# zhang-tao-whu/DVIS_Plus

Hardware: AMD Instinct MI355X
Metric: frames/sec DVIS++ R50 offline, 720p T=30 synthetic (higher is better)
Workload: dtype f32 (storage, accumulation, results; the segmenter's dense layers - R50 convolutions from 128 channels on, pixel-decoder projections and FPN output convolution, the deformable encoder's projections and FFN, the decoder's key / value projections - multiply each fp32 operand as two f16 terms on the f1

## Files before the change

### dvis_plus_amd/csrc/gemm_x3.hip

```cpp
#define DVIS_X3_DMA_MUBUF 1
#include "dvis_common.h"
#include "x3_common.h"

#include <stdlib.h>

namespace {

template <int KS>
__device__ __forceinline__ void load_x(const float *x, int64_t ldx, int64_t row, int g, float s, h8 *xh, h8 *xl,
                                       const float *addp = nullptr) {
  const float *p = x + row * ldx + 8 * g;
  f4 raw[2 * KS];
#pragma unroll
  for (int S = 0; S < KS; ++S) raw[2 * S] = *(const f4 *)(p + 16 * S), raw[2 * S + 1] = *(const f4 *)(p + 16 * S + 4);
  if (addp != nullptr) {
#pragma unroll
    for (int S = 0; S < KS; ++S) raw[2 * S] += *(const f4 *)(addp + 16 * S), raw[2 * S + 1] += *(const f4 *)(addp + 16 * S + 4);
  }
#pragma unroll
  for (int S = 0; S < KS; ++S) split8(raw[2 * S], raw[2 * S + 1], s, xh[S], xl[S]);
}

__device__ __forceinline__ void store_block(char *scr, int lane, const f4 *v, float *dst, int64_t ld, int rows_valid,
                                            const float *radd = nullptr, int64_t ldr = 0) {
// ... 16 lines not shown
  const float *res;
  int64_t ldres;
  const float *gamma, *beta;
  float eps;
  const float *pos;
  int64_t pos_rows;
  float *out, *out2;
  int64_t ldo;
  float inv;
  int relu;
  const float *radd;
  int *flag;
  int tag;
};

template <int NB, bool LN, bool EX = false>
__device__ __forceinline__ void epilogue(f16v *acc, const EpiArgs &e, const float *cb, const float *cg, const float *cbeta, char *scr,
                                         int lane, int64_t tok0, int64_t M, int col0 = 0) {
  const int j = lane & 31, g = lane >> 5;
  const int64_t tok = tok0 + j < M ? tok0 + j : M - 1;
  const int rows_valid = M - tok0 < 32 ? (int)(M - tok0) : 32;
  constexpr int N = 32 * NB;
  float mean = 0.f, rstd = 1.f;
  if constexpr (LN) {
    const float *rp = e.res + tok * e.ldres + 4 * g;
    f4 r[2][4];
    auto fetch = [&](int nb, f4 *dst) {
#pragma unroll
      for (int q = 0; q < 4; ++q) dst[q] = *(const f4 *)(rp + 32 * nb + 8 * q);
    };
    fetch(0, r[0]);
    float sum = 0.f;
#pragma unroll
// ... 25 lines not shown
    rstd = rsqrtf(sq * (1.f / N) + e.eps);
  }
  float chk = 0.f;
  const float *pr = nullptr;
  f4 pv[2][4];
  auto fetch_pos = [&](int nb, f4 *dst) {
#pragma unroll
    for (int q = 0; q < 4; ++q) dst[q] = *(const f4 *)(pr + 32 * nb + 8 * q);
  };
  if constexpr (LN) {
    if (e.pos != nullptr) {
      pr = e.pos + (tok % e.pos_rows) * N + 4 * g;
      fetch_pos(0, pv[0]);
    }
  }
#pragma unroll
  for (int nb = 0; nb < NB; ++nb) {
    f4 v[4];
    if constexpr (LN) {
      if (e.pos != nullptr && nb + 1 < NB) fetch_pos(nb + 1, pv[(nb + 1) & 1]);
    }
#pragma unroll
    for (int q = 0; q < 4; ++q) {
      const int n = 32 * nb + 8 * q + 4 * g;
      if constexpr (LN) {
        const f4 ga = *(const f4 *)(cg + n), be = *(const f4 *)(cbeta + n);
#pragma unroll
        for (int i = 0; i < 4; ++i) v[q][i] = (acc[nb][4 * q + i] - mean) * rstd * ga[i] + be[i];
      } else {
        const f4 b = *(const f4 *)(cb + n);
#pragma unroll
        for (int i = 0; i < 4; ++i) {
          const float t = acc[nb][4 * q + i] * e.inv + b[i];
          chk = __builtin_fmaf(t, 0.f, chk);
          if constexpr (EX)
            v[q][i] = e.relu == 1 ? x3_relu(t) : e.relu == 2 ? 0.5f * t * (1.f + erff(t * 0.70710678118654752440f)) : t;
          else
            v[q][i] = e.relu ? x3_relu(t) : t;
        }
      }
    }
    if constexpr (!EX)
      store_block(scr, lane, v, e.out + tok0 * e.ldo + col0 + 32 * nb, e.ldo, rows_valid);
    else
      store_block(scr, lane, v, e.out + tok0 * e.ldo + col0 + 32 * nb, e.ldo, rows_valid,
                  e.radd ? e.radd + tok0 * e.ldres + col0 + 32 * nb : nullptr, e.ldres);
    if constexpr (LN) {
      if (e.pos != nullptr) {
#pragma unroll
        for (int q = 0; q < 4; ++q) v[q] += pv[nb & 1][q];
        store_block(scr, lane, v, e.out2 + tok0 * e.ldo + 32 * nb, e.ldo, rows_valid);
      }
    }
  }
  if constexpr (!LN) {
// ... 153 lines not shown
          products(stage, acc, xh + 2 * half, xl + 2 * half);
        }
      }
      if (tok0 < M) epilogue<NB, LN, EX>(acc, e, cst + pass * 32 * NB, cst + ntot, cst + ntot + 32 * NB, scr, lane, tok0, M, pass * 32 * NB);
    }
    rowp = nrowp;
  }
}

struct FfnArgs {
  const float *b1;
  float inv1, hscale;
  int HB;
};

__global__ __launch_bounds__(kThreads) void x3_ffn_kernel(const float *__restrict__ x, int64_t ldx, int64_t M,
                                                          const void *__restrict__ wp, float xscale, FfnArgs f, EpiArgs e) {
  extern __shared__ __attribute__((aligned(1024))) char lds[];
  constexpr int KS = 16;
  const int wave = threadIdx.x >> 6, lane = threadIdx.x & 63, j = lane & 31, g = lane >> 5;
  const int64_t ntiles = (M + kTileTok - 1) / kTileTok;
  const int64_t my = blockIdx.x < ntiles ? (ntiles - blockIdx.x + gridDim.x - 1) / gridDim.x : 0;
  const int per_tile = 8 * f.HB;
  Ring<8> ring;
  ring.start(wp, lds, per_tile, (int)(my * per_tile), wave, lane);
  char *scr = lds + kStages * Ring<8>::kItemBytes + wave * kScratch;
  float *b1s = (float *)(lds + kStages * Ring<8>::kItemBytes + kWaves * kScratch);
  for (int i = threadIdx.x; i < 128 * f.HB; i += kThreads) b1s[i] = f.b1[i];
  float *cst = b1s + 128 * f.HB;
  for (int i = threadIdx.x; i < 256; i += kThreads) cst[i] = e.bias[i], cst[256 + i] = e.gamma[i], cst[512 + i] = e.beta[i];
  __syncthreads();
  for (int64_t tile = blockIdx.x; tile < ntiles; tile += gridDim.x) {
    const int64_t tok0 = tile * kTileTok + wave * 32;
    const int64_t row = tok0 + j < M ? tok0 + j : M - 1;
    h8 xh[KS], xl[KS];
    load_x<KS>(x, ldx, row, g, xscale, xh, xl);
    f16v acc2[8];
#pragma unroll
    for (int nb = 0; nb < 8; ++nb)
#pragma unroll
      for (int i = 0; i < 16; ++i) acc2[nb][i] = 0.f;
    for (int hb = 0; hb < f.HB; ++hb) {
      f16v acc1[4];
#pragma unroll
      for (int t = 0; t < 4; ++t)
// ... 22 lines not shown
        mma_item<16, 1, 8>(stage, lane, acc1 + c, xh, xl, [&](int i) { ring.piece(i); }, [&](int t) {
          if (c > 0) convert(c - 1, t);
        });
      }
#pragma unroll
      for (int c = 0; c < 4; ++c) {
        const char *stage = ring.wait(false);
        ring.begin_periodic();
        if (c == 0) {
          mma_item<2, 8, 8>(stage, lane, acc2, hh, hl, [&](int i) { ring.piece(i); }, [&](int t) { convert(3, t); });
        } else {
          mma_item<2, 8, 8>(stage, lane, acc2, hh + 2 * c, hl + 2 * c, [&](int i) { ring.piece(i); });
        }
      }
    }
    if (tok0 < M) epilogue<8, true>(acc2, e, cst, cst + 256, cst + 512, scr, lane, tok0, M);
  }
}

__global__ void x3_ffn_pack_kernel(const float *w1, int64_t ldw1, const float *w2, int64_t ldw2, int H, float s1, float s2,
                                   _Float16 *out, int64_t fragments) {
  const int64_t idx = (int64_t)blockIdx.x * blockDim.x + threadIdx.x;
  if (idx >= fragments) return;
  const int lane = idx & 63;
  int64_t t = idx >> 6;
  const int fr = t & 15;
  t >>= 4;
  const int item = t & 7, hb = t >> 3;
  _Float16 *o = out + (((int64_t)hb * 8 + item) * 16 + fr) * 1024 + lane * 8;
  if (item < 4) {
    x3_pack_fragment(w1, ldw1, H, 256, 128 * hb + 32 * item + (lane & 31), 0, fr, lane >> 5, s1, o, o + 512);
  } else {
    const int s = fr >> 3, nb = fr & 7;
    x3_pack_fragment(w2, ldw2, 256, H, 32 * nb + (lane & 31), 1, 8 * hb + 2 * (item - 4) + s, lane >> 5, s2, o, o + 512);
  }
}

int x3_grid(int64_t ntiles) {
  const int cus = dvis_x3_persistent_cus();
  return (int)(ntiles < cus ? ntiles : cus);
}

float x3_pow2(int e) { return ldexpf(1.f, e); }

template <typename Kern, typename... Args>
int x3_launch(Kern kern, DvisLdsOptIn *opted, size_t lds_bytes, int64_t M, hipStream_t st, const char *what, Args... args) {
  const int rc = dvis_lds_opt_in((const void *)kern, lds_bytes, opted, what);
  if (rc != DVIS_OK) return rc;
  const int64_t ntiles = (M + kTileTok - 1) / kTileTok;
  hipLaunchKernelGGL(kern, dim3(x3_grid(ntiles)), dim3(kThreads), lds_bytes, st, args...);
// ... 202 lines not shown
DVIS_EXPORT int64_t dvis_x3_ffn_packed_bytes(int K, int H, int N) {
  if (K != 256 || N != 256 || H <= 0 || H % 128 != 0 || H > 4096) return -1;
  return (int64_t)(H / 128) * 8 * Ring<8>::kItemBytes;
}

DVIS_EXPORT int dvis_x3_ffn_pack(const float *w1, int64_t ldw1, const float *w2, int64_t ldw2, int K, int H, int N, int w1exp,
                                 int w2exp, void *packed, void *stream) {
  DVIS_REQUIRE(w1 && w2 && packed, "dvis_x3_ffn_pack: null operand");
  DVIS_REQUIRE(dvis_x3_ffn_packed_bytes(K, H, N) > 0, "dvis_x3_ffn_pack: needs K = N = 256, H %% 128 == 0 (K %d, H %d, N %d)", K, H, N);
  const int64_t fragments = (int64_t)(H / 128) * 8 * 16 * 64;
  hipLaunchKernelGGL(x3_ffn_pack_kernel, dim3((unsigned)((fragments + 255) / 256)), dim3(256), 0, (hipStream_t)stream, w1, ldw1,
                     w2, ldw2, H, x3_pow2(w1exp), x3_pow2(w2exp), (_Float16 *)packed, fragments);
  return dvis_check_launch("dvis_x3_ffn_pack");
}

DVIS_EXPORT int dvis_x3_ffn_ln(const float *x, int64_t ldx, int64_t M, int K, int H, int N, const void *wp, int xexp, int w1exp,
                               int hexp, int w2exp, const float *b1, const float *b2, const float *gamma, const float *beta,
                               float eps, const float *pos, int64_t pos_rows, float *out, float *out2, int64_t ldo,
                               void *stream) {
  DVIS_REQUIRE(dvis_x3_ffn_packed_bytes(K, H, N) > 0, "dvis_x3_ffn_ln: needs K = N = 256, H %% 128 == 0 (K %d, H %d, N %d)", K, H, N);
  DVIS_REQUIRE(b1 && b2 && gamma && beta, "dvis_x3_ffn_ln: biases, gamma, beta are required");
  DVIS_REQUIRE(pos == nullptr || (out2 && pos_rows > 0 && (uintptr_t)pos % 16 == 0 && (uintptr_t)out2 % 16 == 0),
               "dvis_x3_ffn_ln: pos needs out2, pos_rows > 0 and 16-byte alignment");
  const int rc = x3_check_common(x, ldx, M, wp, out, ldo);
  if (rc != DVIS_OK) return rc;
  if (M == 0) return DVIS_OK;
  EpiArgs e = {};
  e.bias = b2, e.res = x, e.ldres = ldx, e.gamma = gamma, e.beta = beta, e.eps = eps, e.pos = pos, e.pos_rows = pos_rows;
  e.out = out, e.out2 = out2, e.ldo = ldo, e.inv = x3_pow2(-(hexp + w2exp));
  const X3Guard gd = dvis_x3_guard();
  e.flag = gd.flag, e.tag = gd.tag;
  FfnArgs f = {b1, x3_pow2(-(xexp + w1exp)), x3_pow2(hexp), H / 128};
  static DvisLdsOptIn opted;
  return x3_launch(x3_ffn_kernel, &opted, kStages * Ring<8>::kItemBytes + kWaves * kScratch + (size_t)(H + 3 * 256) * 4, M,
                   (hipStream_t)stream, "dvis_x3_ffn_ln", x, ldx, M, wp, x3_pow2(xexp), f, e);
}
```

### dvis_plus_amd/functions.py

```python
import collections
import ctypes
import math
import os
import threading

import torch
from torch.autograd import Function
from torch.autograd.function import once_differentiable

from . import cpu_ops, derived, native
from .cpu_ops import ms_deform_attn_core_pytorch


def _torch_path(op, x, why):
    if os.environ.get("DVIS_STRICT", "1") != "0" and x.is_cuda and not torch.is_grad_enabled():
        raise RuntimeError(f"DVIS_STRICT: {op} would run its torch formulation on a GPU tensor ({why}; shape "
                           f"{tuple(x.shape)}, dtype {x.dtype}, contiguous {x.is_contiguous()})")


class no_autocast:

    def __enter__(self):
        import contextlib
        self._stack = contextlib.ExitStack()
# ... 1406 lines not shown
            ctypes.c_void_p(x2.data_ptr()), ldx, x2.shape[0], K, ctypes.c_void_p(buf.data_ptr()), N,
            X3_XEXP if xexp is None else xexp, wexp, native.dev_ptr(bias.detach(), "bias"), ctypes.c_void_p(r2.data_ptr()), ldr,
            native.dev_ptr(norm.weight.detach(), "gamma"), native.dev_ptr(norm.bias.detach(), "beta"), float(norm.eps),
            None if pos is None else ctypes.c_void_p(pos.data_ptr()), pos_rows, ctypes.c_void_p(out.data_ptr()),
            None if out2 is None else ctypes.c_void_p(out2.data_ptr()), N, native.stream_ptr(x.device)), "dvis_x3_linear_ln")
    return out if out2 is None else (out, out2)


def x3_ffn_ok(x, lin1, lin2):
    K, H, N = lin1.weight.shape[1], lin1.weight.shape[0], lin2.weight.shape[0]
    return (x.is_cuda and x.dtype == torch.float32 and not torch.is_grad_enabled() and x.shape[-1] == K
            and lin2.weight.shape[1] == H and lin1.bias is not None and lin2.bias is not None
            and native.lib().dvis_x3_ffn_packed_bytes(K, H, N) > 0)


def x3_ffn_ln(x, lin1, lin2, norm, pos=None, xexp=None, hexp=None):
    w1, w2 = lin1.weight, lin2.weight
    H, K = w1.shape
    N = w2.shape[0]
    x2, ldx = _x3_rows(x, "x")

    def make():
        a, b = w1.detach().contiguous(), w2.detach().contiguous()
        e1, e2 = _x3_wexp(a), _x3_wexp(b)
        buf = torch.empty(native.lib().dvis_x3_ffn_packed_bytes(K, H, N), dtype=torch.uint8, device=a.device)
        with torch.cuda.device(a.device):
            native.check(native.lib().dvis_x3_ffn_pack(ctypes.c_void_p(a.data_ptr()), K, ctypes.c_void_p(b.data_ptr()), H, K, H,
                                                       N, e1, e2, ctypes.c_void_p(buf.data_ptr()),
                                                       native.stream_ptr(a.device)), "dvis_x3_ffn_pack")
        return buf, e1, e2
    buf, e1, e2 = _x3_cache(w1, [w1, w2], make, kind="ffn")
    out = torch.empty((*x.shape[:-1], N), dtype=torch.float32, device=x.device)
    pos, pos_rows, out2 = _x3_pos(pos, x, N)
    with torch.cuda.device(x.device):
        native.check(native.lib().dvis_x3_ffn_ln(
            ctypes.c_void_p(x2.data_ptr()), ldx, x2.shape[0], K, H, N, ctypes.c_void_p(buf.data_ptr()),
            X3_XEXP if xexp is None else xexp, e1, X3_XEXP if hexp is None else hexp, e2,
            native.dev_ptr(lin1.bias.detach(), "b1"), native.dev_ptr(lin2.bias.detach(), "b2"),
            native.dev_ptr(norm.weight.detach(), "gamma"), native.dev_ptr(norm.bias.detach(), "beta"), float(norm.eps),
            None if pos is None else ctypes.c_void_p(pos.data_ptr()), pos_rows, ctypes.c_void_p(out.data_ptr()),
            None if out2 is None else ctypes.c_void_p(out2.data_ptr()), N, native.stream_ptr(x.device)), "dvis_x3_ffn_ln")
    return out if out2 is None else (out, out2)


def maps_to_tokens(maps, affines=None, pos=None):
    affines = affines or [None] * len(maps)
    N, C = maps[0].shape[:2]
    if not all(m.is_cuda and m.dtype == torch.float32 and m.is_contiguous() for m in maps) or torch.is_grad_enabled():
        _torch_path("maps_to_tokens", maps[0], "needs contiguous fp32 NCHW maps")
        maps = [m if a is None else m * a[0].view(N, C, 1, 1) + a[1].view(N, C, 1, 1) for m, a in zip(maps, affines)]
        out = torch.cat([m.flatten(2).transpose(1, 2) for m in maps], 1)
        return out if pos is None else (out, out + pos.reshape(1, -1, C))
    S = sum(m.shape[2] * m.shape[3] for m in maps)
    out = torch.empty((N, S, C), dtype=torch.float32, device=maps[0].device)
    out_pos = pp = None
    if pos is not None:
# ... 1089 lines not shown
```

### dvis_plus_amd/native.py

```python
import ctypes
import os

import torch

_HERE = os.path.dirname(os.path.abspath(__file__))
LIB_PATH = os.environ.get("DVIS_HIP_LIB") or os.path.join(_HERE, "lib", "libdvis_hip.so")

F32, F64, F16, BF16 = 0, 1, 2, 3
_DTYPE = {torch.float32: F32, torch.float64: F64, torch.float16: F16, torch.bfloat16: BF16}

_c = ctypes
_i, _i64, _p, _f = _c.c_int, _c.c_int64, _c.c_void_p, _c.c_float

SIGNATURES = {
    "dvis_last_error": (_c.c_char_p, []),
    "dvis_version": (_i, []),
    "dvis_msda_forward": (_i, [_i, _p, _p, _p, _p, _p, _i, _i, _i, _i, _i, _i, _i, _p, _p]),
    "dvis_msda_backward": (_i, [_i, _p, _p, _p, _p, _p, _p, _i, _i, _i, _i, _i, _i, _i, _p, _p, _p, _p]),
    "dvis_msda_backward_det_ws_bytes": (_i64, [_i, _i, _i, _i]),
    "dvis_msda_backward_det": (_i, [_p, _p, _p, _p, _p, _p, _i, _i, _i, _i, _i, _i, _i, _p, _p, _p, _p, _p]),
    "dvis_msda_fused_forward": (_i, [_p, _p, _p, _p, _i, _p, _i64, _p, _i64, _i, _i, _i, _i, _i, _i, _i, _p, _p, _p]),
    "dvis_msda_fused_forward_pos": (_i, [_p, _p, _p, _p, _i, _p, _i64, _p, _i64, _p, _p, _i64, _i, _i, _i, _i, _i, _i, _i,
                                         _p, _p, _p]),
    "dvis_msda_fused_forward_h": (_i, [_i, _p, _p, _p, _p, _i, _p, _i64, _p, _i64, _i, _i, _i, _i, _i, _i, _i, _p, _p, _p]),
# ... 71 lines not shown
    "dvis_x3_tile_linear_qkv": (_i, [_p, _i64, _i64, _i, _p, _i, _i, _i, _p, _i, _i, _f, _p, _p]),
    "dvis_attention_x3_packed": (_i, [_p, _p, _p, _i, _i, _i, _p]),
    "dvis_x3_rows_image_bytes": (_i64, [_i64, _i]),
    "dvis_x3_rows_image": (_i, [_p, _i64, _i64, _i, _i, _p, _p]),
    "dvis_layernorm_rows_image": (_i, [_p, _p, _p, _i64, _i, _f, _i, _p, _p]),
    "dvis_x3_tile_pack_order": (_i, [_p, _i64, _i, _i, _i, _i, _p, _p]),
    "dvis_x3_tile_linear_image": (_i, [_p, _i64, _i, _p, _i, _i, _i, _p, _i, _p, _i64, _p, _i64, _p, _i, _p]),
    "dvis_x3_tile_linear_qkv_image": (_i, [_p, _i64, _i, _p, _i, _i, _i, _p, _i, _i, _f, _p, _p]),
    "dvis_attention_x3_packed_image": (_i, [_p, _p, _i, _i, _i, _i, _p]),
    "dvis_x3_tile_linear": (_i, [_p, _i64, _i64, _i, _p, _i, _i, _i, _p, _i, _p, _i64, _p, _i64, _p]),
    "dvis_x3_linear_res": (_i, [_p, _i64, _i64, _i, _p, _i, _i, _i, _p, _i, _p, _i64, _p, _i64, _p]),
    "dvis_x3_linear_add": (_i, [_p, _i64, _i64, _i, _p, _i, _i, _i, _p, _i64, _p, _i, _p, _i64, _p]),
    "dvis_x3_linear_ln": (_i, [_p, _i64, _i64, _i, _p, _i, _i, _i, _p, _p, _i64, _p, _p, _f, _p, _i64, _p, _p, _i64, _p]),
    "dvis_x3_ffn_packed_bytes": (_i64, [_i, _i, _i]),
    "dvis_x3_ffn_pack": (_i, [_p, _i64, _p, _i64, _i, _i, _i, _i, _i, _p, _p]),
    "dvis_x3_ffn_ln": (_i, [_p, _i64, _i64, _i, _i, _i, _p, _i, _i, _i, _i, _p, _p, _p, _p, _f, _p, _i64, _p, _p, _i64, _p]),
    "dvis_conv1x1_x3_supported": (_i, [_i, _i, _i64, _i64, _i64]),
    "dvis_conv1x1_x3_packed_bytes": (_i64, [_i, _i]),
    "dvis_conv1x1_x3_pack": (_i, [_p, _i, _i, _i, _p, _p]),
    "dvis_conv_x3_gn_fold_supported": (_i, [_i, _i, _i64]),
    "dvis_conv1x1_x3": (_i, [_p, _p, _p, _p, _p, _i, _i, _i, _i, _i, _i, _i, _i, _i, _p, _p, _p, _i, _p]),
    "dvis_conv1x1_x3_dual": (_i, [_p, _p, _p, _p, _p, _p, _i, _i, _i, _i, _i, _i, _i, _i, _i, _i, _i, _i, _p]),
    "dvis_conv3x3_x3_packed_bytes": (_i64, [_i, _i]),
    "dvis_conv3x3_x3_pack": (_i, [_p, _i, _i, _i, _p, _p]),
    "dvis_conv3x3_x3": (_i, [_p, _p, _p, _p, _p, _i, _i, _i, _i, _i, _i, _i, _i, _i, _p]),
    "dvis_bneck_x3_supported": (_i, [_i64, _i, _i]),
    "dvis_bneck_x3_image_bytes": (_i64, [_i64, _i, _i]),
    "dvis_bneck_x3_packed_bytes": (_i64, [_i, _i]),
    "dvis_bneck_x3_pack": (_i, [_p, _p, _p, _p, _i, _i, _i, _p, _p]),
    "dvis_bneck_x3": (_i, [_p, _p, _p, _p, _p, _p, _p, _p, _p, _i, _i, _i, _i, _i, _i, _i, _p]),
    "dvis_conv1x1_x3_image": (_i, [_p, _p, _p, _p, _i, _i, _i, _i, _i, _i, _i, _i, _p]),
# ... 69 lines not shown
```

### dvis_plus_amd/pixel_decoder.py

```python
import math
import os
import warnings

import torch
import torch.nn.functional as F
from torch import nn
from torch.nn.init import constant_, normal_, xavier_uniform_

from . import derived, functions as Fn
from .d2 import configurable
from .registry import SEM_SEG_HEADS_REGISTRY, ShapeSpec

_POS_IN_KERNEL = os.environ.get("DVIS_MSDA_POS", "0") == "1"
_MSDA_SLOTS = int(os.environ.get("DVIS_MSDA_SLOTS", "0") or 0)
_MSDA_HM = os.environ.get("DVIS_MSDA_HM", "0") == "1"


def _is_power_of_2(n):
    if (not isinstance(n, int)) or (n < 0):
        raise ValueError("invalid input for _is_power_of_2: {} (type: {})".format(n, type(n)))
    return (n & (n - 1) == 0) and n != 0


class PositionEmbeddingSine(nn.Module):
# ... 86 lines not shown
                pad = width - w.shape[0]
                if pad:
                    w = torch.cat([w, w.new_zeros(pad, w.shape[1])], 0)
                    b = torch.cat([b, b.new_zeros(pad)], 0)
            w, b = w.contiguous(), b.contiguous()
            rows = w.shape[0] if slot else 3 * M * LP
            return w, b, slot, w[:rows], b[:rows]
        return self._fused.get([so.weight, so.bias, aw.weight, aw.bias], make, (_MSDA_SLOTS,))

    def _fast_path_ok(self, query, reference_points, input_padding_mask):
        d = self.d_model // self.n_heads
        return (not torch.is_grad_enabled() and query.is_cuda and query.dtype in (torch.float32, torch.float16, torch.bfloat16)
                and input_padding_mask is None and reference_points.shape[-1] == 2 and d in (32, 64)
                and (self.n_levels, self.n_points) in ((1, 4), (3, 4), (4, 4)))

    def forward(self, query, reference_points, input_flatten, input_spatial_shapes, input_level_start_index,
                input_padding_mask=None, spatial_shapes_py=None, query_pos=None, post=None):
        if post is not None:
            out = self._forward(query, reference_points, input_flatten, input_spatial_shapes, input_level_start_index,
                                input_padding_mask, spatial_shapes_py, query_pos, post)
            if isinstance(out, tuple):
                return out[0]
            return out + post[0] if post[1] is None else Fn.add_layer_norm(out, post[0], post[1])
        return self._forward(query, reference_points, input_flatten, input_spatial_shapes, input_level_start_index,
                             input_padding_mask, spatial_shapes_py, query_pos, None)

    def _forward(self, query, reference_points, input_flatten, input_spatial_shapes, input_level_start_index,
                 input_padding_mask, spatial_shapes_py, query_pos, post):
        N, Len_q, _ = query.shape
        N, Len_in, _ = input_flatten.shape
        M, L, P = self.n_heads, self.n_levels, self.n_points
        fast = self._fast_path_ok(query, reference_points, input_padding_mask)
        lowp = query.dtype != torch.float32 or torch.is_autocast_enabled()
        hm = fast and _MSDA_HM and input_flatten.is_contiguous() and not lowp
        x3 = fast and Fn.x3_on() and not lowp and not hm and not _MSDA_SLOTS and Fn.x3_ok(input_flatten, self.d_model, self.d_model) \
            and Fn.x3_ok(query, 3 * M * L * P, self.d_model)
        if x3:
            value = Fn.linear(input_flatten, self.value_proj.weight, self.value_proj.bias, tall=True).view(N, Len_in, M, -1)
        elif hm:
            value = Fn.gemm_nt(input_flatten.view(N * Len_in, self.d_model), self.value_proj.weight.detach(),
                               self.value_proj.bias.detach(), head_major=self.d_model // M).view(M, N, Len_in, -1)
        else:
            value = Fn.linear(input_flatten, self.value_proj.weight, self.value_proj.bias, tall=True)
            if input_padding_mask is not None:
                value = value.masked_fill(input_padding_mask[..., None], float(0))
            value = value.view(N, Len_in, M, self.d_model // M)
        if fast:
            w, b, slot, w_rows, b_rows = self._fused_projection()
            o_off, l_off = ((L * P, 0) if _MSDA_SLOTS == 2 else (0, 2 * L * P)) if slot else (0, M * L * P * 2)
            po = pl = None
            if lowp and slot:
                raise RuntimeError("DVIS_MSDA_SLOTS is an fp32-only layout experiment")
            if query_pos is not None and query_pos.shape[0] == 1 and _POS_IN_KERNEL and not lowp:
                pp = Fn.linear(query_pos[0], w)
                po, pl = pp[:, o_off:], pp[:, l_off:]
            elif query_pos is not None and not (x3 and query_pos.shape[0] == 1 and query.dim() == 3 and self.d_model == 256):
                query = query + query_pos
                query_pos = None
            if x3 and query_pos is not None and po is None:
                proj = Fn.x3_linear(query, w_rows, b_rows, xadd=query_pos).view(N * Len_q, -1)
            elif x3:
                proj = Fn.x3_linear(query.reshape(N * Len_q, self.d_model), w_rows, b_rows)
            else:
                proj = Fn.linear(query.reshape(N * Len_q, self.d_model), w, b, tall=True)
            ref = reference_points if reference_points.is_contiguous() else reference_points.contiguous()
            output = Fn.msda_fused_forward(value, input_spatial_shapes, input_level_start_index, ref,
                                           proj[:, o_off:], proj[:, l_off:], L, P, shapes_host=spatial_shapes_py,
                                           pos_offsets=po, pos_logits=pl, head_stride=slot, value_head_major=hm)
            if x3 and post is not None and post[1] is None and post[0].shape[:-1] == output.shape[:-1] and post[0].dtype == torch.float32:
                return (Fn.linear(output, self.output_proj.weight, self.output_proj.bias, tall=True, residual=post[0]),)
            if x3 and post is not None and post[1] is not None and Fn.x3_ok(output, self.d_model, self.d_model, ln=True) \
                    and post[0].shape == output.shape and post[0].dtype == torch.float32 and post[1].weight is not None:
                return (Fn.x3_linear_ln(output, self.output_proj.weight, self.output_proj.bias, post[0], post[1]),)
            if x3:
# ... 31 lines not shown
        self.self_attn = MSDeformAttn(d_model, n_levels, n_heads, n_points)
        self.norm1 = nn.LayerNorm(d_model)
        self.linear1 = nn.Linear(d_model, d_ffn)
        self.linear2 = nn.Linear(d_ffn, d_model)
        self.norm2 = nn.LayerNorm(d_model)
        self.dropout_p = dropout

    def pos_in_projection(self, src, pos):
        a = self.self_attn
        return bool(Fn.x3_on() and pos is not None and pos.dim() == 3 and pos.shape[0] == 1 and src.dim() == 3 and src.is_cuda
                    and src.dtype == torch.float32 and not torch.is_grad_enabled() and not torch.is_autocast_enabled()
                    and not _POS_IN_KERNEL and not _MSDA_SLOTS and not _MSDA_HM and a.d_model == 256
                    and 3 * a.n_heads * a.n_levels * a.n_points in (128, 192, 256, 288) and a.d_model // a.n_heads in (32, 64)
                    and (a.n_levels, a.n_points) in ((1, 4), (3, 4), (4, 4)))

    def forward(self, src, pos, reference_points, spatial_shapes, level_start_index, padding_mask=None,
                shapes_py=None, query=None, emit_next_query=False):
        pos_in_proj = self.pos_in_projection(src, pos)
        if query is not None and not pos_in_proj:
            src = self.self_attn(query, reference_points, src, spatial_shapes, level_start_index, padding_mask,
                                 spatial_shapes_py=shapes_py, post=(src, self.norm1))
        else:
            src = self.self_attn(src, reference_points, src, spatial_shapes, level_start_index, padding_mask,
                                 spatial_shapes_py=shapes_py, query_pos=pos, post=(src, self.norm1))
        if Fn.x3_on() and Fn.x3_ffn_ok(src, self.linear1, self.linear2) and self.norm2.weight is not None:
            with_pos = emit_next_query and pos is not None and pos.shape[0] == 1 and src.dim() == 3 and not pos_in_proj
            r = Fn.x3_ffn_ln(src, self.linear1, self.linear2, self.norm2, pos=pos if with_pos else None)
            return r if with_pos or not emit_next_query else (r, None)
        src2 = Fn.linear(Fn.linear_relu(src, self.linear1, tall=True), self.linear2.weight, self.linear2.bias, tall=True)
        if emit_next_query and pos is not None and pos.shape[0] == 1:
            return Fn.add_layer_norm(src2, src, self.norm2, pos=pos)
        out = Fn.add_layer_norm(src2, src, self.norm2)
        return (out, None) if emit_next_query else out


class MSDeformAttnTransformerEncoder(nn.Module):
    def __init__(self, encoder_layer_factory, num_layers):
        super().__init__()
        self.layers = nn.ModuleList([encoder_layer_factory() for _ in range(num_layers)])
# ... 15 lines not shown
        return reference_points[:, :, None] * valid_ratios[:, None]

    def reference_points_unpadded(self, shapes_py, device):
        key = (tuple(shapes_py), str(device))
        if key not in self._ref_cache:
            vr = torch.ones(1, len(shapes_py), 2, device=device)
            self._ref_cache[key] = self.get_reference_points(shapes_py, vr, device).contiguous()
        return self._ref_cache[key]

    def forward(self, src, spatial_shapes, level_start_index, valid_ratios=None, pos=None, padding_mask=None,
                shapes_py=None, query0=None):
        if valid_ratios is None:
            reference_points = self.reference_points_unpadded(shapes_py, src.device)
        else:
            reference_points = self.get_reference_points(spatial_shapes.tolist(), valid_ratios, src.device)
        output, query = src, query0
        for i, layer in enumerate(self.layers):
            last = i + 1 == len(self.layers)
            r = layer(output, pos, reference_points, spatial_shapes, level_start_index, padding_mask,
                      shapes_py=shapes_py, query=query, emit_next_query=not last)
            output, query = (r, None) if last else r
        return output


class MSDeformAttnTransformerEncoderOnly(nn.Module):
    def __init__(self, d_model=256, nhead=8, num_encoder_layers=6, dim_feedforward=1024, dropout=0.1,
                 activation="relu", num_feature_levels=4, enc_n_points=4):
        super().__init__()
        self.d_model, self.nhead = d_model, nhead
        self.encoder = MSDeformAttnTransformerEncoder(
            lambda: MSDeformAttnTransformerEncoderLayer(d_model, dim_feedforward, dropout, activation,
                                                        num_feature_levels, nhead, enc_n_points),
            num_encoder_layers)
        self.level_embed = nn.Parameter(torch.Tensor(num_feature_levels, d_model))
        self._shape_cache = {}
        self._reset_parameters()
# ... 225 lines not shown
```

### include/dvis_hip.h

```cpp
#ifndef DVIS_HIP_H
#define DVIS_HIP_H

#include <stdint.h>

#ifdef __cplusplus
extern "C" {
#endif

enum { DVIS_F32 = 0, DVIS_F64 = 1, DVIS_F16 = 2, DVIS_BF16 = 3 };

enum {
  DVIS_OK = 0,
  DVIS_E_ARG = -1,
  DVIS_E_LAUNCH = -2,
  DVIS_E_UNSUPPORTED = -3
};

const char *dvis_last_error(void);
int dvis_version(void);

int dvis_msda_forward(int dtype, const void *value, const int64_t *shapes, const int64_t *level_start,
                      const void *loc, const void *w, int N, int S, int M, int D, int L, int Lq, int P,
                      void *out, void *stream);

// ... 226 lines not shown
int dvis_bneck_x3(const void *a1, const float *res, const float *x2, const void *packed, const float *b2, const float *b3,
                  const float *b1, float *y, void *out, int N, int H, int W, int xexp, int e2, int e3, int e1, void *stream);
int dvis_conv1x1_x3_image(const float *x, const void *packed, const float *bias, void *image, int N, int C, int H, int W, int xexp,
                          int wexp, int oexp, int relu, void *stream);
int64_t dvis_conv_x3_image_bytes(int64_t N, int C, int H, int W);
int dvis_conv_x3_pack_image(const float *w, int K, int C, int taps, int wexp, void *packed, void *stream);
int dvis_conv_x3_image(const void *ximg, const float *x, const void *packed, const float *bias, const float *res, float *y, void *image,
                       int N, int C, int K, int H, int W, int stride, int taps, int xexp, int wexp, int oexp, int relu, void *stream,
                       double *gn_part);
int dvis_upsample_add_image(const float *lateral, const float *lat_scale, const float *lat_shift, const float *top, void *image, int N,
                            int C, int H, int W, int h, int w, int oexp, void *stream);
int dvis_x3_ffn_pack(const float *W1, int64_t ldw1, const float *W2, int64_t ldw2, int K, int H, int N, int w1exp, int w2exp,
                     void *packed, void *stream);
int dvis_x3_ffn_ln(const float *x, int64_t ldx, int64_t M, int K, int H, int N, const void *packed, int xexp, int w1exp,
                   int hexp, int w2exp, const float *b1, const float *b2, const float *gamma, const float *beta, float eps,
                   const float *pos, int64_t pos_rows, float *out, float *out2, int64_t ldo, void *stream);

int dvis_pan_pair_hist(const int32_t *gt, const int32_t *pred, const int32_t *gt_table, int Ng, int Np, int T, int64_t HW,
                       int64_t *out, int64_t *bad, void *stream);
int dvis_sem_confusion(const int32_t *gt, const int32_t *pred, int64_t n, int num_class, int64_t *out, int64_t *bad, void *stream);
int dvis_video_consistency(const int32_t *gt, const int32_t *pred, int T, int64_t HW, const int32_t *ks, int nk, int64_t *gt_const,
                           int64_t *both_const, void *stream);

int dvis_rle_encode(const uint8_t *masks, int64_t N, int H, int W, int phase, int64_t *trans, int64_t *area, const int64_t *toff,
                    const int64_t *moff, int32_t *bnd, uint32_t *runs, void *stream);
int dvis_rle_strings(const uint32_t *runs, const int64_t *run_off, int64_t N, const int64_t *str_off, int64_t *lens, uint8_t *chars,
                     void *stream);
int dvis_rle_decode(const int32_t *ends, const int64_t *run_off, int64_t N, int H, int W, uint8_t *out, void *stream);
int dvis_track_intersections(const uint8_t *pred, int64_t pred_stride, int P, const uint8_t *gt, int64_t gt_stride, int G, int T,
                             int64_t HW, int accumulate, int64_t *out, void *stream);

// ... 25 lines not shown
```

Before: 414.3.

## Chain next encoder layer's value and offset projections into the FFN+LN kernel

The deformable encoder's FFN+LayerNorm kernel now optionally computes the next layer's value projection (from the normalized output) and sampling-offset/attention projection (from output plus positional embedding) while the output tile is still in registers. This removes two separate GEMM launches per encoder layer and the re-read of the layer output from memory. In exchange the FFN kernel streams extra packed weight items per tile and carries more live state. The Python encoder loop passes the precomputed projections to the next layer through a new 'pre' argument. The path is on by default behind DVIS_ENC_CHAIN.

```diff
diff --git a/dvis_plus_amd/csrc/gemm_x3.hip b/dvis_plus_amd/csrc/gemm_x3.hip
--- a/dvis_plus_amd/csrc/gemm_x3.hip
+++ b/dvis_plus_amd/csrc/gemm_x3.hip
@@ -3,6 +3,7 @@
 #include "x3_common.h"
 
 #include <stdlib.h>
+#include <type_traits>
 
 namespace {
 
@@ -54,9 +55,16 @@
   int tag;
 };
 
-template <int NB, bool LN, bool EX = false>
+struct ChainFrags {
+  h8 *vh, *vl;
+  const float *cpos;
+  int64_t cpos_rows;
+  float xscale;
+};
+
+template <int NB, bool LN, bool EX = false, bool CH = false>
 __device__ __forceinline__ void epilogue(f16v *acc, const EpiArgs &e, const float *cb, const float *cg, const float *cbeta, char *scr,
-                                         int lane, int64_t tok0, int64_t M, int col0 = 0) {
+                                         int lane, int64_t tok0, int64_t M, int col0 = 0, const ChainFrags *ch = nullptr) {
   const int j = lane & 31, g = lane >> 5;
   const int64_t tok = tok0 + j < M ? tok0 + j : M - 1;
   const int rows_valid = M - tok0 < 32 ? (int)(M - tok0) : 32;
@@ -112,11 +120,24 @@
       fetch_pos(0, pv[0]);
     }
   }
+  const float *cpr = nullptr;
+  f4 cpv[2][4];
+  auto fetch_cpos = [&](int nb, f4 *dst) {
+#pragma unroll
+    for (int q = 0; q < 4; ++q) dst[q] = *(const f4 *)(cpr + 32 * nb + 8 * q);
+  };
+  if constexpr (CH) {
+    cpr = ch->cpos + (tok % ch->cpos_rows) * N + 4 * g;
+    fetch_cpos(0, cpv[0]);
+  }
 #pragma unroll
   for (int nb = 0; nb < NB; ++nb) {
     f4 v[4];
     if constexpr (LN) {
       if (e.pos != nullptr && nb + 1 < NB) fetch_pos(nb + 1, pv[(nb + 1) & 1]);
+    }
+    if constexpr (CH) {
+      if (nb + 1 < NB) fetch_cpos(nb + 1, cpv[(nb + 1) & 1]);
     }
 #pragma unroll
     for (int q = 0; q < 4; ++q) {
@@ -137,6 +158,14 @@
             v[q][i] = e.relu ? x3_relu(t) : t;
         }
       }
+    }
+    if constexpr (CH) {
+#pragma unroll
+      for (int u = 0; u < 2; ++u) split8(v[2 * u], v[2 * u + 1], ch->xscale, ch->vh[2 * nb + u], ch->vl[2 * nb + u]);
+#pragma unroll
+      for (int q = 0; q < 4; ++q)
+#pragma unroll
+        for (int i = 0; i < 4; ++i) acc[nb][4 * q + i] = v[q][i] + cpv[nb & 1][q][i];
     }
     if constexpr (!EX)
       store_block(scr, lane, v, e.out + tok0 * e.ldo + col0 + 32 * nb, e.ldo, rows_valid);
@@ -320,14 +349,26 @@
   int HB;
 };
 
+struct ChainArgs {
+  const float *bv, *bo;
+  const float *pos;
+  int64_t pos_rows;
+  float *value, *proj;
+  int64_t ldv, ldp;
+  float invv, invo;
+};
+constexpr int kChainV = 8, kChainO = 9, kChainItems = kChainV + kChainO;
+
+template <bool CHAIN>
 __global__ __launch_bounds__(kThreads) void x3_ffn_kernel(const float *__restrict__ x, int64_t ldx, int64_t M,
-                                                          const void *__restrict__ wp, float xscale, FfnArgs f, EpiArgs e) {
+                                                          const void *__restrict__ wp, float xscale, FfnArgs f, EpiArgs e,
+                                                          ChainArgs ca) {
   extern __shared__ __attribute__((aligned(1024))) char lds[];
   constexpr int KS = 16;
   const int wave = threadIdx.x >> 6, lane = threadIdx.x & 63, j = lane & 31, g = lane >> 5;
   const int64_t ntiles = (M + kTileTok - 1) / kTileTok;
   const int64_t my = blockIdx.x < ntiles ? (ntiles - blockIdx.x + gridDim.x - 1) / gridDim.x : 0;
-  const int per_tile = 8 * f.HB;
+  const int per_tile = 8 * f.HB + (CHAIN ? kChainItems : 0);
   Ring<8> ring;
   ring.start(wp, lds, per_tile, (int)(my * per_tile), wave, lane);
   char *scr = lds + kStages * Ring<8>::kItemBytes + wave * kScratch;
@@ -335,6 +376,11 @@
   for (int i = threadIdx.x; i < 128 * f.HB; i += kThreads) b1s[i] = f.b1[i];
   float *cst = b1s + 128 * f.HB;
   for (int i = threadIdx.x; i < 256; i += kThreads) cst[i] = e.bias[i], cst[256 + i] = e.gamma[i], cst[512 + i] = e.beta[i];
+  float *cbs = cst + 768;
+  if constexpr (CHAIN) {
+    for (int i = threadIdx.x; i < 32 * kChainItems; i += kThreads)
+      cbs[i] = i < 256 ? (ca.bv ? ca.bv[i] : 0.f) : (ca.bo ? ca.bo[i - 256] : 0.f);
+  }
   __syncthreads();
   for (int64_t tile = blockIdx.x; tile < ntiles; tile += gridDim.x) {
     const int64_t tok0 = tile * kTileTok + wave * 32;
@@ -387,7 +433,78 @@
         }
       }
     }
-    if (tok0 < M) epilogue<8, true>(acc2, e, cst, cst + 256, cst + 512, scr, lane, tok0, M);
+    if constexpr (!CHAIN) {
+      if (tok0 < M) epilogue<8, true>(acc2, e, cst, cst + 256, cst + 512, scr, lane, tok0, M);
+    } else {
+      int ln = lane;
+      asm volatile("" : "+v"(ln));
+      const ChainFrags cf = {xh, xl, ca.pos, ca.pos_rows, xscale};
+      epilogue<8, true, false, true>(acc2, e, cst, cst + 256, cst + 512, scr, ln, tok0, M, 0, &cf);
+      const int rows_valid = M - tok0 < 32 ? (int)(M - tok0) : 32;
+      const int cj = ln & 31, cg = ln >> 5, sw = (cj >> 1) & 7, jr0 = ln >> 3, pp = ln & 7;
+      char *wslot = scr + cj * 128;
+      const int64_t offv = jr0 * ca.ldv + 4 * pp, offo = jr0 * ca.ldp + 4 * pp;
+      float chk = 0.f;
+      f16v cur, prev;
+      float *pdst = nullptr;
+      int64_t pld = 0;
+      float pinv = 0.f;
+      const float *pb = cbs;
+      f4 ro[2];
+      auto emit = [&](int t) {
+        if (t < 4) {
+          const f4 b = *(const f4 *)(pb + 8 * t + 4 * cg);
+          f4 v;
+#pragma unroll
+          for (int i = 0; i < 4; ++i) {
+            v[i] = prev[4 * t + i] * pinv + b[i];
+            chk = __builtin_fmaf(v[i], 0.f, chk);
+          }
+          asm volatile("" : "+v"(chk));
+          *(f4 *)(wslot + (((2 * t + cg) ^ sw) << 4)) = v;
+        } else if (t < 9) {
+          if (t == 4) __builtin_amdgcn_wave_barrier();
+          if (t > 4 && 8 * (t - 5) + jr0 < rows_valid) *(f4 *)(pdst + 8 * (t - 5) * pld) = ro[(t - 5) & 1];
+          if (t < 8) {
+            const int jr = 8 * (t - 4) + jr0;
+            ro[(t - 4) & 1] = *(const f4 *)(scr + jr * 128 + ((pp ^ ((jr >> 1) & 7)) << 4));
+          } else {
+            __builtin_amdgcn_wave_barrier();
+          }
+        }
+      };
+      auto item = [&](auto have_prev, const h8 *fh, const h8 *fl) {
+        const char *stage = ring.wait(false);
+        ring.begin_periodic();
+#pragma unroll
+        for (int i = 0; i < 16; ++i) cur[i] = 0.f;
+        mma_item<16, 1, 8>(stage, lane, &cur, fh, fl, [&](int i) { ring.piece(i); }, [&](int t) {
+          if constexpr (decltype(have_prev)::value) emit(t);
+        });
+        prev = cur;
+      };
+      for (int p = 0; p < kChainV; ++p) {
+        if (p == 0)
+          item(std::false_type{}, xh, xl);
+        else
+          item(std::true_type{}, xh, xl);
+        pdst = ca.value + tok0 * ca.ldv + 32 * p + offv, pld = ca.ldv, pinv = ca.invv, pb = cbs + 32 * p;
+      }
+#pragma unroll
+      for (int S = 0; S < KS; ++S) {
+        const f16v &a = acc2[S >> 1];
+        const int o = 8 * (S & 1);
+        split8(f4{a[o], a[o + 1], a[o + 2], a[o + 3]}, f4{a[o + 4], a[o + 5], a[o + 6], a[o + 7]}, xscale, xh[S], xl[S]);
+      }
+      for (int p = 0; p < kChainO; ++p) {
+        item(std::true_type{}, xh, xl);
+        pdst = ca.proj + tok0 * ca.ldp + 32 * p + offo, pld = ca.ldp, pinv = ca.invo, pb = cbs + 256 + 32 * p;
+      }
+#pragma unroll
+      for (int t = 0; t < 9; ++t) emit(t);
+      __builtin_amdgcn_wave_barrier();
+      if (e.flag != nullptr && chk != chk) atomicCAS(e.flag, 0, e.tag);
+    }
   }
 }
 
@@ -407,6 +524,18 @@
     const int s = fr >> 3, nb = fr & 7;
     x3_pack_fragment(w2, ldw2, 256, H, 32 * nb + (lane & 31), 1, 8 * hb + 2 * (item - 4) + s, lane >> 5, s2, o, o + 512);
   }
+}
+
+__global__ void x3_ffn_chain_pack_kernel(const float *wv, int64_t ldwv, const float *wo, int64_t ldwo, float sv, float so,
+                                         _Float16 *out, int64_t fragments) {
+  const int64_t idx = (int64_t)blockIdx.x * blockDim.x + threadIdx.x;
+  if (idx >= fragments) return;
+  const int lane = idx & 63, fr = (idx >> 6) & 15, item = (int)(idx >> 10);
+  _Float16 *o = out + ((int64_t)item * 16 + fr) * 1024 + lane * 8;
+  if (item < kChainV)
+    x3_pack_fragment(wv, ldwv, 32 * kChainV, 256, 32 * item + (lane & 31), 1, fr, lane >> 5, sv, o, o + 512);
+  else
+    x3_pack_fragment(wo, ldwo, 32 * kChainO, 256, 32 * (item - kChainV) + (lane & 31), 1, fr, lane >> 5, so, o, o + 512);
 }
 
 int x3_grid(int64_t ntiles) {
@@ -639,10 +768,31 @@
   return dvis_check_launch("dvis_x3_ffn_pack");
 }
 
+DVIS_EXPORT int64_t dvis_x3_ffn_chain_packed_bytes(int K, int H, int N, int Nv, int No) {
+  if (dvis_x3_ffn_packed_bytes(K, H, N) <= 0 || Nv != 32 * kChainV || No != 32 * kChainO) return 0;
+  return dvis_x3_ffn_packed_bytes(K, H, N) + (int64_t)kChainItems * Ring<8>::kItemBytes;
+}
+
+DVIS_EXPORT int dvis_x3_ffn_chain_pack(const float *w1, int64_t ldw1, const float *w2, int64_t ldw2, const float *wv, int64_t ldwv,
+                                       const float *wo, int64_t ldwo, int K, int H, int N, int Nv, int No, int w1exp, int w2exp,
+                                       int wvexp, int woexp, void *packed, void *stream) {
+  DVIS_REQUIRE(wv && wo && packed, "dvis_x3_ffn_chain_pack: null operand");
+  DVIS_REQUIRE(dvis_x3_ffn_chain_packed_bytes(K, H, N, Nv, No) > 0,
+               "dvis_x3_ffn_chain_pack: needs K = N = Nv = 256, No = 288, H %% 128 == 0 (K %d, H %d, N %d, Nv %d, No %d)", K, H, N, Nv, No);
+  DVIS_REQUIRE(wvexp >= -60 && wvexp <= 60 && woexp >= -60 && woexp <= 60, "dvis_x3_ffn_chain_pack: wvexp = %d, woexp = %d", wvexp, woexp);
+  const int rc = dvis_x3_ffn_pack(w1, ldw1, w2, ldw2, K, H, N, w1exp, w2exp, packed, stream);
+  if (rc != DVIS_OK) return rc;
+  const int64_t fragments = (int64_t)kChainItems * 16 * 64;
+  hipLaunchKernelGGL(x3_ffn_chain_pack_kernel, dim3((unsigned)((fragments + 255) / 256)), dim3(256), 0, (hipStream_t)stream, wv, ldwv,
+                     wo, ldwo, x3_pow2(wvexp), x3_pow2(woexp), (_Float16 *)((char *)packed + dvis_x3_ffn_packed_bytes(K, H, N)), fragments);
+  return dvis_check_launch("dvis_x3_ffn_chain_pack");
+}
+
 DVIS_EXPORT int dvis_x3_ffn_ln(const float *x, int64_t ldx, int64_t M, int K, int H, int N, const void *wp, int xexp, int w1exp,
                                int hexp, int w2exp, const float *b1, const float *b2, const float *gamma, const float *beta,
                                float eps, const float *pos, int64_t pos_rows, float *out, float *out2, int64_t ldo,
-                               void *stream) {
+                               void *stream, const void *chain, int wvexp, int woexp, const float *bv, const float *bo,
+                               const float *cpos, int64_t cpos_rows, float *value, int64_t ldv, float *proj, int64_t ldp) {
   DVIS_REQUIRE(dvis_x3_ffn_packed_bytes(K, H, N) > 0, "dvis_x3_ffn_ln: needs K = N = 256, H %% 128 == 0 (K %d, H %d, N %d)", K, H, N);
   DVIS_REQUIRE(b1 && b2 && gamma && beta, "dvis_x3_ffn_ln: biases, gamma, beta are required");
   DVIS_REQUIRE(pos == nullptr || (out2 && pos_rows > 0 && (uintptr_t)pos % 16 == 0 && (uintptr_t)out2 % 16 == 0),
@@ -656,7 +806,18 @@
   const X3Guard gd = dvis_x3_guard();
   e.flag = gd.flag, e.tag = gd.tag;
   FfnArgs f = {b1, x3_pow2(-(xexp + w1exp)), x3_pow2(hexp), H / 128};
+  if (chain != nullptr) {
+    DVIS_REQUIRE(cpos && cpos_rows > 0 && value && proj, "dvis_x3_ffn_ln: the chained form needs cpos, cpos_rows > 0, value and proj");
+    DVIS_REQUIRE((uintptr_t)chain % 16 == 0 && (uintptr_t)cpos % 16 == 0 && (uintptr_t)value % 16 == 0 && (uintptr_t)proj % 16 == 0 &&
+                     ldv % 4 == 0 && ldp % 4 == 0 && ldv >= 32 * kChainV && ldp >= 32 * kChainO,
+                 "dvis_x3_ffn_ln: chained operands must be 16-byte aligned with row strides %% 4 == 0, ldv >= 256, ldp >= 288");
+    ChainArgs ca = {bv, bo, cpos, cpos_rows, value, proj, ldv, ldp, x3_pow2(-(xexp + wvexp)), x3_pow2(-(xexp + woexp))};
+    static DvisLdsOptIn opted_chain;
+    return x3_launch(x3_ffn_kernel<true>, &opted_chain,
+                     kStages * Ring<8>::kItemBytes + kWaves * kScratch + (size_t)(H + 3 * 256 + 32 * kChainItems) * 4, M,
+                     (hipStream_t)stream, "dvis_x3_ffn_ln", x, ldx, M, chain, x3_pow2(xexp), f, e, ca);
+  }
   static DvisLdsOptIn opted;
-  return x3_launch(x3_ffn_kernel, &opted, kStages * Ring<8>::kItemBytes + kWaves * kScratch + (size_t)(H + 3 * 256) * 4, M,
-                   (hipStream_t)stream, "dvis_x3_ffn_ln", x, ldx, M, wp, x3_pow2(xexp), f, e);
-}
+  return x3_launch(x3_ffn_kernel<false>, &opted, kStages * Ring<8>::kItemBytes + kWaves * kScratch + (size_t)(H + 3 * 256) * 4, M,
+                   (hipStream_t)stream, "dvis_x3_ffn_ln", x, ldx, M, wp, x3_pow2(xexp), f, e, ChainArgs{});
+}
diff --git a/dvis_plus_amd/functions.py b/dvis_plus_amd/functions.py
--- a/dvis_plus_amd/functions.py
+++ b/dvis_plus_amd/functions.py
@@ -1444,11 +1444,63 @@
             and native.lib().dvis_x3_ffn_packed_bytes(K, H, N) > 0)
 
 
-def x3_ffn_ln(x, lin1, lin2, norm, pos=None, xexp=None, hexp=None):
+ENC_CHAIN = os.environ.get("DVIS_ENC_CHAIN", "1") != "0"
+
+
+def x3_ffn_chain_ok(lin1, lin2, Nv, No):
+    K, H, N = lin1.weight.shape[1], lin1.weight.shape[0], lin2.weight.shape[0]
+    return bool(ENC_CHAIN and native.lib().dvis_x3_ffn_chain_packed_bytes(K, H, N, Nv, No) > 0)
+
+
+def x3_ffn_ln(x, lin1, lin2, norm, pos=None, xexp=None, hexp=None, chain=None):
     w1, w2 = lin1.weight, lin2.weight
     H, K = w1.shape
     N = w2.shape[0]
     x2, ldx = _x3_rows(x, "x")
+    if chain is not None:
+        if pos is not None:
+            raise RuntimeError("x3_ffn_ln: chain and pos are not served together")
+        wv, bv, wo, bo, cpos = chain
+        cpos_rows = cpos.numel() // N
+        if cpos.dtype != torch.float32 or not cpos.is_cuda or cpos_rows * N != cpos.numel() or cpos_rows == 0 \
+                or (x.dim() == 3 and x.shape[1] != cpos_rows) or x.dim() not in (2, 3):
+            raise RuntimeError("x3_ffn_ln: chain needs a float32 GPU (S, C) embedding for x of shape (N, S, C) (or (M, C): row t "
+                               "takes embedding row t mod S)")
+        Nv, No = wv.shape[0], wo.shape[0]
+        if wv.shape[1] != N or wo.shape[1] != N or wv.dtype != torch.float32 or wo.dtype != torch.float32:
+            raise RuntimeError("x3_ffn_ln: the chained weights must be float32 (Nv, C) and (No, C)")
+        nbytes = native.lib().dvis_x3_ffn_chain_packed_bytes(K, H, N, Nv, No)
+        if nbytes <= 0:
+            raise RuntimeError(f"x3_ffn_ln: the chained projections {tuple(wv.shape)}, {tuple(wo.shape)} are not served")
+
+        def make_chain():
+            a, b = w1.detach().contiguous(), w2.detach().contiguous()
+            v, o = wv.detach().contiguous(), wo.detach().contiguous()
+            e1, e2, ev, eo = _x3_wexp(a), _x3_wexp(b), _x3_wexp(v), _x3_wexp(o)
+            buf = torch.empty(nbytes, dtype=torch.uint8, device=a.device)
+            with torch.cuda.device(a.device):
+                native.check(native.lib().dvis_x3_ffn_chain_pack(
+                    ctypes.c_void_p(a.data_ptr()), K, ctypes.c_void_p(b.data_ptr()), H, ctypes.c_void_p(v.data_ptr()), N,
+                    ctypes.c_void_p(o.data_ptr()), N, K, H, N, Nv, No, e1, e2, ev, eo, ctypes.c_void_p(buf.data_ptr()),
+                    native.stream_ptr(a.device)), "dvis_x3_ffn_chain_pack")
+            return buf, e1, e2, ev, eo
+        buf, e1, e2, ev, eo = _x3_cache(w1, [w1, w2, wv, wo], make_chain, kind="ffn_chain")
+        cpos = cpos.contiguous()
+        out = torch.empty((*x.shape[:-1], N), dtype=torch.float32, device=x.device)
+        value = torch.empty((*x.shape[:-1], Nv), dtype=torch.float32, device=x.device)
+        proj = torch.empty((*x.shape[:-1], No), dtype=torch.float32, device=x.device)
+        xe = X3_XEXP if xexp is None else xexp
+        with torch.cuda.device(x.device):
+            native.check(native.lib().dvis_x3_ffn_ln(
+                ctypes.c_void_p(x2.data_ptr()), ldx, x2.shape[0], K, H, N, ctypes.c_void_p(buf.data_ptr()),
+                xe, e1, X3_XEXP if hexp is None else hexp, e2,
+                native.dev_ptr(lin1.bias.detach(), "b1"), native.dev_ptr(lin2.bias.detach(), "b2"),
+                native.dev_ptr(norm.weight.detach(), "gamma"), native.dev_ptr(norm.bias.detach(), "beta"), float(norm.eps),
+                None, 0, ctypes.c_void_p(out.data_ptr()), None, N, native.stream_ptr(x.device),
+                ctypes.c_void_p(buf.data_ptr()), ev, eo, None if bv is None else native.dev_ptr(bv.detach(), "bv"),
+                None if bo is None else native.dev_ptr(bo.detach(), "bo"), ctypes.c_void_p(cpos.data_ptr()), cpos_rows,
+                ctypes.c_void_p(value.data_ptr()), Nv, ctypes.c_void_p(proj.data_ptr()), No), "dvis_x3_ffn_ln")
+        return out, value, proj
 
     def make():
         a, b = w1.detach().contiguous(), w2.detach().contiguous()
@@ -1469,7 +1521,8 @@
             native.dev_ptr(lin1.bias.detach(), "b1"), native.dev_ptr(lin2.bias.detach(), "b2"),
             native.dev_ptr(norm.weight.detach(), "gamma"), native.dev_ptr(norm.bias.detach(), "beta"), float(norm.eps),
             None if pos is None else ctypes.c_void_p(pos.data_ptr()), pos_rows, ctypes.c_void_p(out.data_ptr()),
-            None if out2 is None else ctypes.c_void_p(out2.data_ptr()), N, native.stream_ptr(x.device)), "dvis_x3_ffn_ln")
+            None if out2 is None else ctypes.c_void_p(out2.data_ptr()), N, native.stream_ptr(x.device),
+            None, 0, 0, None, None, None, 0, None, 0, None, 0), "dvis_x3_ffn_ln")
     return out if out2 is None else (out, out2)
 
 
diff --git a/dvis_plus_amd/native.py b/dvis_plus_amd/native.py
--- a/dvis_plus_amd/native.py
+++ b/dvis_plus_amd/native.py
@@ -109,7 +109,10 @@
     "dvis_x3_linear_ln": (_i, [_p, _i64, _i64, _i, _p, _i, _i, _i, _p, _p, _i64, _p, _p, _f, _p, _i64, _p, _p, _i64, _p]),
     "dvis_x3_ffn_packed_bytes": (_i64, [_i, _i, _i]),
     "dvis_x3_ffn_pack": (_i, [_p, _i64, _p, _i64, _i, _i, _i, _i, _i, _p, _p]),
-    "dvis_x3_ffn_ln": (_i, [_p, _i64, _i64, _i, _i, _i, _p, _i, _i, _i, _i, _p, _p, _p, _p, _f, _p, _i64, _p, _p, _i64, _p]),
+    "dvis_x3_ffn_ln": (_i, [_p, _i64, _i64, _i, _i, _i, _p, _i, _i, _i, _i, _p, _p, _p, _p, _f, _p, _i64, _p, _p, _i64, _p,
+                            _p, _i, _i, _p, _p, _p, _i64, _p, _i64, _p, _i64]),
+    "dvis_x3_ffn_chain_packed_bytes": (_i64, [_i, _i, _i, _i, _i]),
+    "dvis_x3_ffn_chain_pack": (_i, [_p, _i64, _p, _i64, _p, _i64, _p, _i64, _i, _i, _i, _i, _i, _i, _i, _i, _i, _p, _p]),
     "dvis_conv1x1_x3_supported": (_i, [_i, _i, _i64, _i64, _i64]),
     "dvis_conv1x1_x3_packed_bytes": (_i64, [_i, _i]),
     "dvis_conv1x1_x3_pack": (_i, [_p, _i, _i, _i, _p, _p]),
diff --git a/dvis_plus_amd/pixel_decoder.py b/dvis_plus_amd/pixel_decoder.py
--- a/dvis_plus_amd/pixel_decoder.py
+++ b/dvis_plus_amd/pixel_decoder.py
@@ -124,28 +124,42 @@
                 and input_padding_mask is None and reference_points.shape[-1] == 2 and d in (32, 64)
                 and (self.n_levels, self.n_points) in ((1, 4), (3, 4), (4, 4)))
 
+    def chain_projections(self):
+        _, _, _, w_rows, b_rows = self._fused_projection()
+        return self.value_proj.weight, self.value_proj.bias, w_rows, b_rows
+
     def forward(self, query, reference_points, input_flatten, input_spatial_shapes, input_level_start_index,
-                input_padding_mask=None, spatial_shapes_py=None, query_pos=None, post=None):
+                input_padding_mask=None, spatial_shapes_py=None, query_pos=None, post=None, pre=None):
         if post is not None:
             out = self._forward(query, reference_points, input_flatten, input_spatial_shapes, input_level_start_index,
-                                input_padding_mask, spatial_shapes_py, query_pos, post)
+                                input_padding_mask, spatial_shapes_py, query_pos, post, pre)
             if isinstance(out, tuple):
                 return out[0]
             return out + post[0] if post[1] is None else Fn.add_layer_norm(out, post[0], post[1])
         return self._forward(query, reference_points, input_flatten, input_spatial_shapes, input_level_start_index,
-                             input_padding_mask, spatial_shapes_py, query_pos, None)
+                             input_padding_mask, spatial_shapes_py, query_pos, None, pre)
+
+    def _x3_projections_ok(self, query, input_flatten, reference_points, input_padding_mask):
+        M, L, P = self.n_heads, self.n_levels, self.n_points
+        lowp = query.dtype != torch.float32 or torch.is_autocast_enabled()
+        return bool(self._fast_path_ok(query, reference_points, input_padding_mask) and Fn.x3_on() and not lowp
+                    and not (_MSDA_HM and input_flatten.is_contiguous()) and not _MSDA_SLOTS
+                    and Fn.x3_ok(input_flatten, self.d_model, self.d_model) and Fn.x3_ok(query, 3 * M * L * P, self.d_model))
 
     def _forward(self, query, reference_points, input_flatten, input_spatial_shapes, input_level_start_index,
-                 input_padding_mask, spatial_shapes_py, query_pos, post):
+                 input_padding_mask, spatial_shapes_py, query_pos, post, pre=None):
         N, Len_q, _ = query.shape
         N, Len_in, _ = input_flatten.shape
         M, L, P = self.n_heads, self.n_levels, self.n_points
         fast = self._fast_path_ok(query, reference_points, input_padding_mask)
         lowp = query.dtype != torch.float32 or torch.is_autocast_enabled()
         hm = fast and _MSDA_HM and input_flatten.is_contiguous() and not lowp
-        x3 = fast and Fn.x3_on() and not lowp and not hm and not _MSDA_SLOTS and Fn.x3_ok(input_flatten, self.d_model, self.d_model) \
-            and Fn.x3_ok(query, 3 * M * L * P, self.d_model)
-        if x3:
+        x3 = self._x3_projections_ok(query, input_flatten, reference_points, input_padding_mask)
+        if pre is not None and not x3:
+            raise RuntimeError("MSDeformAttn: chained projections (pre) are served on the split-f16 path only")
+        if pre is not None:
+            value = pre[0].view(N, Len_in, M, -1)
+        elif x3:
             value = Fn.linear(input_flatten, self.value_proj.weight, self.value_proj.bias, tall=True).view(N, Len_in, M, -1)
         elif hm:
             value = Fn.gemm_nt(input_flatten.view(N * Len_in, self.d_model), self.value_proj.weight.detach(),
@@ -167,7 +181,9 @@
             elif query_pos is not None and not (x3 and query_pos.shape[0] == 1 and query.dim() == 3 and self.d_model == 256):
                 query = query + query_pos
                 query_pos = None
-            if x3 and query_pos is not None and po is None:
+            if pre is not None:
+                proj, po, pl = pre[1].view(N * Len_q, -1), None, None
+            elif x3 and query_pos is not None and po is None:
                 proj = Fn.x3_linear(query, w_rows, b_rows, xadd=query_pos).view(N * Len_q, -1)
             elif x3:
                 proj = Fn.x3_linear(query.reshape(N * Len_q, self.d_model), w_rows, b_rows)
@@ -229,15 +245,31 @@
                     and 3 * a.n_heads * a.n_levels * a.n_points in (128, 192, 256, 288) and a.d_model // a.n_heads in (32, 64)
                     and (a.n_levels, a.n_points) in ((1, 4), (3, 4), (4, 4)))
 
+    def chains_into(self, nxt, src, pos, reference_points, padding_mask=None):
+        a = nxt.self_attn
+        if not (Fn.ENC_CHAIN and nxt.pos_in_projection(src, pos) and self.norm2.weight is not None
+                and Fn.x3_ffn_ok(src, self.linear1, self.linear2)
+                and a._x3_projections_ok(src, src, reference_points, padding_mask)
+                and a.value_proj.weight._base is None and a.value_proj.weight.shape == (a.d_model, a.d_model)):
+            return False
+        return Fn.x3_ffn_chain_ok(self.linear1, self.linear2, a.d_model, 3 * a.n_heads * a.n_levels * a.n_points)
+
     def forward(self, src, pos, reference_points, spatial_shapes, level_start_index, padding_mask=None,
-                shapes_py=None, query=None, emit_next_query=False):
+                shapes_py=None, query=None, emit_next_query=False, pre=None, chain_next=None):
         pos_in_proj = self.pos_in_projection(src, pos)
-        if query is not None and not pos_in_proj:
+        if pre is not None:
+            src = self.self_attn(src, reference_points, src, spatial_shapes, level_start_index, padding_mask,
+                                 spatial_shapes_py=shapes_py, query_pos=pos, post=(src, self.norm1), pre=pre)
+        elif query is not None and not pos_in_proj:
             src = self.self_attn(query, reference_points, src, spatial_shapes, level_start_index, padding_mask,
                                  spatial_shapes_py=shapes_py, post=(src, self.norm1))
         else:
             src = self.self_attn(src, reference_points, src, spatial_shapes, level_start_index, padding_mask,
                                  spatial_shapes_py=shapes_py, query_pos=pos, post=(src, self.norm1))
+        if chain_next is not None:
+            out, value, proj = Fn.x3_ffn_ln(src, self.linear1, self.linear2, self.norm2,
+                                            chain=(*chain_next.self_attn.chain_projections(), pos))
+            return out, None, (value, proj)
         if Fn.x3_on() and Fn.x3_ffn_ok(src, self.linear1, self.linear2) and self.norm2.weight is not None:
             with_pos = emit_next_query and pos is not None and pos.shape[0] == 1 and src.dim() == 3 and not pos_in_proj
             r = Fn.x3_ffn_ln(src, self.linear1, self.linear2, self.norm2, pos=pos if with_pos else None)
@@ -283,12 +315,18 @@
             reference_points = self.reference_points_unpadded(shapes_py, src.device)
         else:
             reference_points = self.get_reference_points(spatial_shapes.tolist(), valid_ratios, src.device)
-        output, query = src, query0
+        output, query, pre = src, query0, None
         for i, layer in enumerate(self.layers):
             last = i + 1 == len(self.layers)
+            nxt = None if last else self.layers[i + 1]
+            if nxt is not None and not layer.chains_into(nxt, output, pos, reference_points, padding_mask):
+                nxt = None
             r = layer(output, pos, reference_points, spatial_shapes, level_start_index, padding_mask,
-                      shapes_py=shapes_py, query=query, emit_next_query=not last)
-            output, query = (r, None) if last else r
+                      shapes_py=shapes_py, query=query, emit_next_query=not last, pre=pre, chain_next=nxt)
+            if nxt is not None:
+                output, query, pre = r
+            else:
+                (output, query), pre = ((r, None) if last else r), None
         return output
 
 
diff --git a/include/dvis_hip.h b/include/dvis_hip.h
--- a/include/dvis_hip.h
+++ b/include/dvis_hip.h
@@ -264,7 +264,13 @@
                      void *packed, void *stream);
 int dvis_x3_ffn_ln(const float *x, int64_t ldx, int64_t M, int K, int H, int N, const void *packed, int xexp, int w1exp,
                    int hexp, int w2exp, const float *b1, const float *b2, const float *gamma, const float *beta, float eps,
-                   const float *pos, int64_t pos_rows, float *out, float *out2, int64_t ldo, void *stream);
+                   const float *pos, int64_t pos_rows, float *out, float *out2, int64_t ldo, void *stream,
+                   const void *chain, int wvexp, int woexp, const float *bv, const float *bo, const float *cpos, int64_t cpos_rows,
+                   float *value, int64_t ldv, float *proj, int64_t ldp);
+int64_t dvis_x3_ffn_chain_packed_bytes(int K, int H, int N, int Nv, int No);
+int dvis_x3_ffn_chain_pack(const float *W1, int64_t ldw1, const float *W2, int64_t ldw2, const float *Wv, int64_t ldwv, const float *Wo,
+                           int64_t ldwo, int K, int H, int N, int Nv, int No, int w1exp, int w2exp, int wvexp, int woexp, void *packed,
+                           void *stream);
 
 int dvis_pan_pair_hist(const int32_t *gt, const int32_t *pred, const int32_t *gt_table, int Ng, int Np, int T, int64_t HW,
                        int64_t *out, int64_t *bad, void *stream);
```

Result: no change. 415.4, median of 6 (+0.3%).
